# clysto/tinyimgcodec

Hardware: AMD Instinct MI355X
Metric: Mpixels/s encode (DCT+quant kernel) (higher is better)
Workload: dtype f32+f64

## Files before the change

tinyimgcodec_amd/csrc/tic_kernels.hip:

```cpp
#include <hip/hip_runtime.h>
#include <hip/hip_ext.h>
#include <stdint.h>
#include <stdlib.h>
#include <string.h>
#include <type_traits>

#include "tic_hooks.h"
#include "tic_kernels.h"
#include "tic_math.h"

namespace tic {

#define TIC_DPP_QP_XOR1 0xB1
#define TIC_DPP_QP_XOR2 0x4E
#define TIC_DPP_ROW_SHL4 0x104
#define TIC_DPP_ROW_SHR4 0x114

__device__ __forceinline__ uint32_t perm_b32(uint32_t hi_src, uint32_t lo_src, uint32_t sel) {
    return __builtin_amdgcn_perm(hi_src, lo_src, sel);
}

__device__ __forceinline__ void transpose8x8_bytes(uint32_t &lo, uint32_t &hi, int i) {
    uint32_t nhi = (uint32_t)__builtin_amdgcn_update_dpp((int)hi, (int)lo, TIC_DPP_ROW_SHL4, 0xf, 0x5, false);
    uint32_t nlo = (uint32_t)__builtin_amdgcn_update_dpp((int)lo, (int)hi, TIC_DPP_ROW_SHR4, 0xf, 0xa, false);
    lo = nlo;
    hi = nhi;
    uint32_t selB = (i & 2) ? 0x03020706u : 0x05040100u;
    uint32_t plo = (uint32_t)__builtin_amdgcn_mov_dpp((int)lo, TIC_DPP_QP_XOR2, 0xf, 0xf, true);
    uint32_t phi = (uint32_t)__builtin_amdgcn_mov_dpp((int)hi, TIC_DPP_QP_XOR2, 0xf, 0xf, true);
    lo = perm_b32(plo, lo, selB);
    hi = perm_b32(phi, hi, selB);
    uint32_t selC = (i & 1) ? 0x03070105u : 0x06020400u;
    plo = (uint32_t)__builtin_amdgcn_mov_dpp((int)lo, TIC_DPP_QP_XOR1, 0xf, 0xf, true);
    phi = (uint32_t)__builtin_amdgcn_mov_dpp((int)hi, TIC_DPP_QP_XOR1, 0xf, 0xf, true);
    lo = perm_b32(plo, lo, selC);
    hi = perm_b32(phi, hi, selC);
}

__device__ __forceinline__ void transpose8x8_bytes_shfl(uint32_t &lo, uint32_t &hi, int i) {
    uint32_t row[2] = {lo, hi};
    uint32_t col_lo = 0, col_hi = 0;
    int base = (threadIdx.x & 63) & ~7;
    for (int r = 0; r < 8; r++) {
        uint32_t l = __shfl(row[0], base + r, 64), h = __shfl(row[1], base + r, 64);
        uint32_t w = (i < 4) ? l : h;
        uint32_t byte = (w >> (8 * (i & 3))) & 0xffu;
        if (r < 4)
            col_lo |= byte << (8 * r);
        else
            col_hi |= byte << (8 * (r - 4));
    }
    lo = col_lo;
    hi = col_hi;
}

__device__ __forceinline__ void wave_lds_fence() {
    __builtin_amdgcn_fence(__ATOMIC_RELEASE, "wavefront");
    __builtin_amdgcn_wave_barrier();
    __builtin_amdgcn_fence(__ATOMIC_ACQUIRE, "wavefront");
}

__device__ __forceinline__ int reflect_index(int i, int n) {
    if (i < n) return i;
    if (n >= 8) return 2 * (n - 1) - i;
    if (n == 1) return 0;
    int p = 2 * (n - 1), j = i;
    while (j >= p) j -= p;
    return j < n ? j : p - j;
}

constexpr int kWavesPerWG = 4;
constexpr int kLdsStrideDw = 68;
constexpr int kZzStrideB = 144;
constexpr int kLdsWaveBytes = 8 * kLdsStrideDw * 4;

struct Strip {
    int by, bx;
    bool valid;
    size_t oblk;
};

__device__ __forceinline__ void load_block_row(const uint8_t *__restrict__ img, int h, int w, long stride, bool aligned8,
                                               const Strip &s, int i, uint32_t &lo, uint32_t &hi) {
    lo = 0;
    hi = 0;
    if (!s.valid) return;
    int y = reflect_index(s.by * 8 + i, h);
    int x0 = s.bx * 8;
    const uint8_t *p = img + (long)y * stride + x0;
    if (aligned8 && x0 + 8 <= w) {
        uint2 v = *reinterpret_cast<const uint2 *>(p);
        lo = v.x;
        hi = v.y;
    } else {
        const uint8_t *rowp = img + (long)y * stride;
#pragma unroll
        for (int k = 0; k < 8; k++) {
            uint32_t b = rowp[reflect_index(x0 + k, w)];
            if (k < 4)
                lo |= b << (8 * k);
            else
                hi |= b << (8 * (k - 4));
        }
    }
}

__device__ __forceinline__ void transpose8x8_dwords(uint32_t *lds, int b, int i, uint32_t v[8]) {
    uint32_t *blk = lds + b * kLdsStrideDw;
#pragma unroll
    for (int u = 0; u < 8; u++) blk[u * 8 + i] = v[u];
    wave_lds_fence();
    const uint4 *rp = reinterpret_cast<const uint4 *>(blk + i * 8);
    uint4 a = rp[0], c = rp[1];
    v[0] = a.x; v[1] = a.y; v[2] = a.z; v[3] = a.w;
    v[4] = c.x; v[5] = c.y; v[6] = c.z; v[7] = c.w;
    wave_lds_fence();
}

__device__ __forceinline__ void exact_block(uint32_t colLo, uint32_t colHi, uint32_t *lds, int b, int i,
                                         const DctqConsts *__restrict__ C, int q[8]) {
    double c[8];
#pragma unroll
    for (int r = 0; r < 4; r++) {
        c[r] = (double)((int)((colLo >> (8 * r)) & 0xffu) - 128);
        c[r + 4] = (double)((int)((colHi >> (8 * r)) & 0xffu) - 128);
    }
    dct8_exact(c[0], c[1], c[2], c[3], c[4], c[5], c[6], c[7]);
    uint32_t w[8];
#pragma unroll
    for (int k = 0; k < 8; k++) w[k] = (uint32_t)__double2loint(c[k]);
    transpose8x8_dwords(lds, b, i, w);
    uint32_t wh[8];
#pragma unroll
    for (int k = 0; k < 8; k++) wh[k] = (uint32_t)__double2hiint(c[k]);
    transpose8x8_dwords(lds, b, i, wh);
#pragma unroll
    for (int k = 0; k < 8; k++) c[k] = __hiloint2double((int)wh[k], (int)w[k]);
    dct8_exact(c[0], c[1], c[2], c[3], c[4], c[5], c[6], c[7]);
    const double *div = C->div + i * 8;
#pragma unroll
    for (int v = 0; v < 8; v++) {
        q[v] = (int)rint(c[v] / div[v]);
        __builtin_amdgcn_sched_barrier(0);
    }
}

__device__ __forceinline__ void store_zigzag(uint32_t *lds, int b, int i, const uint16_t zz[8], const int q[8],
                                             int16_t *__restrict__ out, const Strip &s) {
    char *blk = reinterpret_cast<char *>(lds) + b * kZzStrideB;
#pragma unroll
    for (int v = 0; v < 8; v++) *reinterpret_cast<int16_t *>(blk + zz[v]) = (int16_t)q[v];
    wave_lds_fence();
    uint4 val = *reinterpret_cast<const uint4 *>(blk + i * 16);
    wave_lds_fence();
    if (s.valid) *reinterpret_cast<uint4 *>(out + s.oblk * 64 + i * 8) = val;
}

__device__ __forceinline__ Strip make_strip(int tile, int ntiles, int tiles_x, int bw, int b) {
    Strip s;
    int ty = tile / tiles_x;
    int tx = tile - ty * tiles_x;
    s.by = ty;
    s.bx = tx * 8 + b;
    s.valid = (tile < ntiles) && (s.bx < bw);
    s.oblk = (size_t)ty * bw + s.bx;
    return s;
}

__global__ __launch_bounds__(kWavesPerWG * 64) void dctq_exact_kernel(DctqArgs a) {
    __shared__ __attribute__((aligned(16))) uint32_t lds_all[kWavesPerWG][kLdsWaveBytes / 4];
    a.img += (long)blockIdx.y * a.frame_stride_in;
    a.out = reinterpret_cast<int16_t *>(reinterpret_cast<char *>(a.out) + (long)blockIdx.y * a.frame_stride_out);
    const int lane = threadIdx.x & 63, wave = threadIdx.x >> 6;
    const int b = lane >> 3, i = lane & 7;
    uint32_t *lds = lds_all[wave];
    int tile = blockIdx.x * kWavesPerWG + wave;
    int ntiles = a.ntiles;
    if (a.rem_mode) {
        const int bh = a.ntiles / a.tiles_x, rw = a.tiles_x - a.fast_tx;
        const int n_right = bh * rw, n_bottom = (bh - a.fast_ty) * a.fast_tx;
        ntiles = 0;
        if (tile < n_right) {
            tile = (tile / rw) * a.tiles_x + a.fast_tx + tile % rw;
            ntiles = a.ntiles;
        } else if (tile < n_right + n_bottom) {
            const int k = tile - n_right;
            tile = (a.fast_ty + k / a.fast_tx) * a.tiles_x + k % a.fast_tx;
            ntiles = a.ntiles;
        }
    }
    Strip s = make_strip(tile, ntiles, a.tiles_x, a.bw, b);
    uint32_t lo, hi;
    load_block_row(a.img, a.h, a.w, a.stride, a.aligned8, s, i, lo, hi);
    transpose8x8_bytes(lo, hi, i);
    int q[8];
    exact_block(lo, hi, lds, b, i, a.consts, q);
    const uint4 zzv = *reinterpret_cast<const uint4 *>(a.consts->zzofs + i * 8);
    uint16_t zz[8] = {(uint16_t)zzv.x, (uint16_t)(zzv.x >> 16), (uint16_t)zzv.y, (uint16_t)(zzv.y >> 16),
                      (uint16_t)zzv.z, (uint16_t)(zzv.z >> 16), (uint16_t)zzv.w, (uint16_t)(zzv.w >> 16)};
    store_zigzag(lds, b, i, zz, q, a.out, s);
}

constexpr int kTWaveBytes = kLdsWaveBytes;
constexpr int kTHalfDw = 272;
constexpr int kZzWaveBytes = 8 * kZzStrideB;
constexpr int kPxBlkBytes = 80;
constexpr int kMaxStripsPerWave = 16;
constexpr int kChunkStrips = 8;

__device__ __forceinline__ void quant_fma(float z, float mul, uint32_t &bits, float &d) {
    const float s = fmaf(z, mul, kMagic);
    bits = __float_as_uint(s);
    const float nr = kMagic - s;
    d = fmaf(z, mul, nr);
}

__device__ __forceinline__ void store16_wt_nt(void *p, const uint4 &v) {
    typedef uint32_t u32x4 __attribute__((ext_vector_type(4)));
    const u32x4 d = {v.x, v.y, v.z, v.w};
    asm volatile("global_store_dwordx4 %0, %1, off sc1 nt" : : "v"(p), "v"(d) : "memory");
}
__device__ __forceinline__ void store16_wt_nt(const void *sbase, uint32_t voff, const uint4 &v) {
    typedef uint32_t u32x4 __attribute__((ext_vector_type(4)));
    const u32x4 d = {v.x, v.y, v.z, v.w};
    asm volatile("global_store_dwordx4 %0, %1, %2 sc1 nt" : : "v"(voff), "v"(d), "s"(sbase) : "memory");
}

constexpr int kMaxStripsPerWave2 = 64;
constexpr int kBatch = 8;
constexpr int kBatchWaveBytes = kBatch * (128 + 64) + 64;

template <int CTRL>
__device__ __forceinline__ double dpp_f64(double x) {
    const int lo = __builtin_amdgcn_mov_dpp(__double2loint(x), CTRL, 0xf, 0xf, true);
    const int hi = __builtin_amdgcn_mov_dpp(__double2hiint(x), CTRL, 0xf, 0xf, true);
    return __hiloint2double(hi, lo);
}

__device__ __forceinline__ int rational_quad(const uint32_t *ldsT, int b, int i, const double *cst_rat) {
#pragma clang fp contract(off)
    const int w = i >> 2, k = i & 3;
    const uint32_t ca = (0x05010300u >> (8 * k)) & 0xffu, cb = (0x06020407u >> (8 * k)) & 0xffu;
    const uint32_t *row = ldsT + w * 128 + 4 * b;
    const float fa = __uint_as_float(row[(ca >> 2) * kTHalfDw + (ca & 3)]);
    const float fb = __uint_as_float(row[(cb >> 2) * kTHalfDw + (cb & 3)]);
    const double K = w ? (kTW3 * 0.5) : (kSq2h * 0.5);
    const double ya = (double)fa * K, yb = (double)fb * K;
    const double p = ya + yb;
    const double s2 = p + dpp_f64<TIC_DPP_QP_XOR1>(p);
    const double o = dpp_f64<TIC_DPP_QP_XOR2>(s2);
    const double E = (k & 1) ? s2 - o : s2 + o;
    const double X = E * ((k & 1) ? (kTW3 * 0.5) : (kSq2h * 0.5));
    const double div = cst_rat[2 * w + (k & 1)], rdiv = cst_rat[4 + 2 * w + (k & 1)];
    return (int)rint(div_rn(X, div, rdiv));
}

__device__ __forceinline__ int rational_slim(uint32_t rowLo, uint32_t rowHi, int i, const double *cst_rat) {
#pragma clang fp contract(off)
    uint32_t lo = perm_b32(rowHi, rowLo, 0x04030700u);
    uint32_t hi = perm_b32(rowHi, rowLo, 0x06050201u);
    transpose8x8_bytes(lo, hi, i);
    const uint32_t tot = __builtin_amdgcn_sad_u8(lo, 0u, __builtin_amdgcn_sad_u8(hi, 0u, 0u));
    const uint32_t sa = __builtin_amdgcn_sad_u8(lo & 0xff0000ffu, 0u, __builtin_amdgcn_sad_u8(hi & 0xff0000ffu, 0u, 0u));
    const int e0 = (int)tot - 1024, e4 = 2 * (int)sa - (int)tot;
    double y0 = (double)e0 * (kSq2h * 0.5);
    double y4 = (double)e4 * (kTW3 * 0.5);
    y0 = y0 + dpp_f64<TIC_DPP_QP_XOR1>(y0);
    y4 = y4 + dpp_f64<TIC_DPP_QP_XOR1>(y4);
    y0 = y0 + dpp_f64<TIC_DPP_QP_XOR2>(y0);
    y4 = y4 + dpp_f64<TIC_DPP_QP_XOR2>(y4);
    const double b0 = dpp_f64<TIC_DPP_ROW_SHL4>(y0), b4 = dpp_f64<TIC_DPP_ROW_SHL4>(y4);
    const double A = (i & 2) ? y4 : y0, B = (i & 2) ? b4 : b0;
    const double E = (i & 1) ? A - B : A + B;
    const double X = E * ((i & 1) ? (kTW3 * 0.5) : (kSq2h * 0.5));
    const double div = cst_rat[i & 3], rdiv = cst_rat[4 + (i & 3)];
    return (int)rint(div_rn(X, div, rdiv));
}
__device__ __forceinline__ unsigned long long wave_redo_block(const uint8_t *px , double *tbuf ,
                                                              const double *cosm, const double *rdiv, const uint16_t *zzofs, int16_t *img16,
                                                              int lane) {
    const int u = lane >> 3, c = lane & 7;
    typedef double d2 __attribute__((ext_vector_type(2)));
    const d2 *mu = reinterpret_cast<const d2 *>(cosm + u * 8), *mc = reinterpret_cast<const d2 *>(cosm + c * 8);
    const d2 m0 = mu[0], m1 = mu[1], m2 = mu[2], m3 = mu[3];
    double x[8];
#pragma unroll
    for (int r = 0; r < 8; r++) x[r] = (double)((int)px[r * 8 + c] - 128);
    double ta = m0.x * x[0], tb = m0.y * x[1];
    ta = fma(m1.x, x[2], ta); tb = fma(m1.y, x[3], tb);
    ta = fma(m2.x, x[4], ta); tb = fma(m2.y, x[5], tb);
    ta = fma(m3.x, x[6], ta); tb = fma(m3.y, x[7], tb);
    tbuf[u * 8 + c] = ta + tb;
    const d2 n0 = mc[0], n1 = mc[1], n2 = mc[2], n3 = mc[3];
    wave_lds_fence();
    const d2 *tu = reinterpret_cast<const d2 *>(tbuf + u * 8);
    const d2 y0 = tu[0], y1 = tu[1], y2 = tu[2], y3 = tu[3];
    double xa = n0.x * y0.x, xb = n0.y * y0.y;
    xa = fma(n1.x, y1.x, xa); xb = fma(n1.y, y1.y, xb);
    xa = fma(n2.x, y2.x, xa); xb = fma(n2.y, y2.y, xb);
    xa = fma(n3.x, y3.x, xa); xb = fma(n3.y, y3.y, xb);
    const double X = xa + xb;
    const double tq = X * rdiv[lane], rq = rint(tq);
    const bool rational = (lane & 0x1b) == 0;
    const bool decided = fabs(tq - rq) < 0.5 - 1e-9;
    if (decided && !rational) img16[zzofs[lane] >> 1] = (int16_t)(int)rq;
    const unsigned long long und = __ballot(!decided && !rational);
    wave_lds_fence();
    return und;
}

__device__ __forceinline__ uint32_t second_level_8(uint32_t colLo, uint32_t colHi, uint32_t *lds, int b, int i, const double *mul64, int q[8]) {
    double c[8];
#pragma unroll
    for (int r = 0; r < 4; r++) {
        c[r] = (double)(int)((colLo >> (8 * r)) & 0xffu);
        c[r + 4] = (double)(int)((colHi >> (8 * r)) & 0xffu);
    }
    dct8_aan(c[0], c[1], c[2], c[3], c[4], c[5], c[6], c[7]);
    c[0] -= 1024.0;
    uint32_t w[8], wh[8];
#pragma unroll
    for (int k = 0; k < 8; k++) w[k] = (uint32_t)__double2loint(c[k]);
    transpose8x8_dwords(lds, b, i, w);
#pragma unroll
    for (int k = 0; k < 8; k++) wh[k] = (uint32_t)__double2hiint(c[k]);
    transpose8x8_dwords(lds, b, i, wh);
#pragma unroll
    for (int k = 0; k < 8; k++) c[k] = __hiloint2double((int)wh[k], (int)w[k]);
    dct8_aan(c[0], c[1], c[2], c[3], c[4], c[5], c[6], c[7]);
    uint32_t und = 0;
#pragma unroll
    for (int v = 0; v < 8; v++) {
        const double t = c[v] * mul64[i * 8 + v], r = rint(t);
        q[v] = (int)r;
        if (!(fabs(t - r) < 0.5 - 1e-9)) und |= 1u << v;
    }
    return und;
}

template <bool kCols>
__global__ __launch_bounds__(kWavesPerWG * 64, 6) __attribute__((amdgpu_num_vgpr(72))) void dctq_strip_kernel(DctqArgs a) {
    __shared__ __attribute__((aligned(16))) uint32_t ldsT_all[kWavesPerWG][kTWaveBytes / 4];
    __shared__ __attribute__((aligned(16))) uint32_t ldsZ_all[kWavesPerWG][kZzWaveBytes / 4];
    __shared__ __attribute__((aligned(16))) unsigned char cst_blk[kStripBlkBytes];
    __shared__ __attribute__((aligned(16))) uint32_t bat_all[kWavesPerWG][kBatchWaveBytes / 4];
    const int lane = threadIdx.x & 63;
    const int wave = __builtin_amdgcn_readfirstlane(threadIdx.x >> 6);
    uint32_t *ldsT = ldsT_all[wave];
    char *ldsZ = reinterpret_cast<char *>(ldsZ_all[wave]);
    const uint16_t *cst_zz = reinterpret_cast<const uint16_t *>(cst_blk + kBlkZz);
    const double *cst_rat = reinterpret_cast<const double *>(cst_blk + kBlkRat);
    uint4 *bat_img = reinterpret_cast<uint4 *>(bat_all[wave]);
    uint2 *bat_pix = reinterpret_cast<uint2 *>(bat_all[wave] + kBatch * 32);
    uint32_t *bat_id = bat_all[wave] + kBatch * 48;
    const DctqConsts *__restrict__ C = a.consts;
    a.img += (long)blockIdx.z * a.frame_stride_in;
    a.out = reinterpret_cast<int16_t *>(reinterpret_cast<char *>(a.out) + (long)blockIdx.z * a.frame_stride_out);

    const int lr = lane >> 3, lb = lane & 7;
    const int b = lane >> 3, i = lane & 7;
    unsigned long long mask_exact = 0;
    uint32_t n_second = 0, n_quad = 0;
    int nE = 0;
    int t_first, n_my;
    const uint32_t st_off = (uint32_t)lane * 16u;
    {
        typedef float f32x4 __attribute__((ext_vector_type(4)));
        typedef uint32_t u32x4 __attribute__((ext_vector_type(4)));
        f32x4 m0, m1;
        f32x4 thr;
        u32x4 zzv;
        u32x4 c_fill;
        {
            constexpr int kPpw = kStripBlkPieces / kWavesPerWG;
            static_assert(kPpw * kWavesPerWG == kStripBlkPieces && kPpw <= 64, "constant block must split evenly over the waves");
            const uint32_t piece = lane < kPpw ? (uint32_t)(wave * kPpw + lane) : (uint32_t)kStripBlkPieces - 1u;
            const uint32_t fo = piece * 16u;
            asm volatile("global_load_dwordx4 v[76:79], %0, %1" : : "v"(fo), "s"(C->strip_blk) : "memory", "v76", "v77", "v78", "v79");
        }
        const uint32_t px_wr = (uint32_t)(uintptr_t)(__attribute__((address_space(3))) char *)(ldsZ + lb * kPxBlkBytes + lr * 8);
        const uint8_t *px_rd = reinterpret_cast<const uint8_t *>(ldsZ + b * kPxBlkBytes + i);
        constexpr int kHalf = kCols ? kTHalfDw : 256;
        const int p1a = kCols ? i : lr, p1b = kCols ? b : lb;
        uint32_t *twA = ldsT + (p1a >> 2) * kHalf + (p1a & 3) + 4 * p1b;
        uint32_t *twB = ldsT + (p1a >> 2) * kHalf + (p1a & 3) + 4 * (p1b ^ 4);
        const uint4 *tr = reinterpret_cast<const uint4 *>(
            __builtin_assume_aligned(ldsT + i * 32 + 4 * (b ^ (4 * ((i >> 1) & 1))), 16));
        const uint32_t ld_off = (uint32_t)(lr * (int)a.stride + lb * 8);

        uint32_t tf, t_lim;
        if (a.team_count > 0) {
            const uint32_t r = blockIdx.y;
            const uint32_t row0 = (uint32_t)((r < 8u ? a.split_lo >> (8u * r) : a.split_hi) & 0xffull);
            const uint32_t row1 = (uint32_t)((r < 7u ? a.split_lo >> (8u * r + 8u) : a.split_hi) & 0xffull);
            tf = (row0 * (uint32_t)a.team_count + blockIdx.x) * kWavesPerWG + (uint32_t)wave;
            t_lim = tf + (row1 - row0) * (uint32_t)a.tstep;
        } else if (a.round_wgs > 0) {
            const uint32_t rho = a.magic_tstep ? __umulhi(blockIdx.x, a.magic_tstep ) : blockIdx.x;
            const uint32_t wl = blockIdx.x - rho * (uint32_t)a.round_wgs;
            const uint32_t base = rho * (uint32_t)a.round_wgs * (uint32_t)a.wg_span;
            tf = base + wl * kWavesPerWG + (uint32_t)wave;
            t_lim = base + (uint32_t)a.round_wgs * (uint32_t)a.wg_span;
        } else {
            tf = blockIdx.x * (uint32_t)a.wg_stride + (uint32_t)wave;
            t_lim = blockIdx.x * (uint32_t)a.wg_stride + (uint32_t)a.wg_span;
        }
        tf = __builtin_amdgcn_readfirstlane(tf);
        const uint32_t nfast = (uint32_t)a.fast_ty * (uint32_t)a.fast_tx;
        const uint32_t t_end = t_lim < nfast ? t_lim : nfast;
        n_my = 0;
        if (tf < t_end) n_my = (a.round_wgs > 0 || a.magic_tstep == 0u) ? (int)((t_end - tf + (uint32_t)a.tstep - 1u) / (uint32_t)a.tstep)
                                                                        : (int)__umulhi(t_end - tf + (uint32_t)a.tstep - 1u, a.magic_tstep);
        if (n_my == 0) tf = 0;
        t_first = (int)tf;
        const uint32_t ty_first = a.magic_fast_tx ? __umulhi(tf, a.magic_fast_tx) : tf;
        int txp = (int)(tf - ty_first * (uint32_t)a.fast_tx);
        uint32_t in_off = ty_first * (uint32_t)(8 * a.stride) + (uint32_t)txp * 64u;
        uint32_t oblk = ty_first * (uint32_t)a.bw + (uint32_t)txp * 8u;
        uint32_t src_off = 0;
        int n_issued = 0;
        const uint8_t *img_s = a.img;
#define TIC_RSV_CLOBBER "memory", "v72", "v73", "v74", "v75", "v76", "v77", "v78", "v79"
#define TIC_LOAD(R, OB)                                                                                      \
    do {                                                                                                     \
        src_off = n_issued < n_my ? in_off : src_off;                                                        \
        OB = oblk;                                                                                           \
        asm volatile("global_load_dwordx2 v[" R "], %0, %1" : : "v"(ld_off), "s"(img_s + src_off) : TIC_RSV_CLOBBER); \
        n_issued++; txp += a.step_tx; in_off += a.in_step32; oblk += a.oblk_step;                            \
        if (__builtin_expect(txp >= a.fast_tx, 0)) { txp -= a.fast_tx; in_off += a.in_wrap32; oblk += a.oblk_wrap; } \
    } while (0)
#define TIC_TAKE_COLS(R, N) asm volatile("s_waitcnt vmcnt(" #N ")\n\tds_write_b64 %0, v[" R "]" : : "v"(px_wr) : TIC_RSV_CLOBBER)
#define TIC_TAKE_ROWS(D, R0, R1, N)                                                                          \
    asm volatile("s_waitcnt vmcnt(" #N ")\n\tv_cvt_f32_ubyte0 %0, v" #R0 "\n\tv_cvt_f32_ubyte1 %1, v" #R0 "\n\tv_cvt_f32_ubyte2 %2, v" #R0 \
                 "\n\tv_cvt_f32_ubyte3 %3, v" #R0 "\n\tv_cvt_f32_ubyte0 %4, v" #R1 "\n\tv_cvt_f32_ubyte1 %5, v" #R1                       \
                 "\n\tv_cvt_f32_ubyte2 %6, v" #R1 "\n\tv_cvt_f32_ubyte3 %7, v" #R1                                                       \
                 : "=v"(D[0]), "=v"(D[1]), "=v"(D[2]), "=v"(D[3]), "=v"(D[4]), "=v"(D[5]), "=v"(D[6]), "=v"(D[7]) : : TIC_RSV_CLOBBER)
        uint32_t ob0, ob1, ob2;
        uint32_t kstrip = 0;
        TIC_LOAD("72:73", ob0);
        TIC_LOAD("74:75", ob1);
        asm volatile("s_waitcnt vmcnt(2)\n\tv_mov_b32 %0, v76\n\tv_mov_b32 %1, v77\n\tv_mov_b32 %2, v78\n\tv_mov_b32 %3, v79"
                     : "=v"(c_fill.x), "=v"(c_fill.y), "=v"(c_fill.z), "=v"(c_fill.w) : : "memory", "v76", "v77", "v78", "v79");
        if (lane < kStripBlkPieces / kWavesPerWG) *reinterpret_cast<u32x4 *>(cst_blk + (wave * (kStripBlkPieces / kWavesPerWG) + lane) * 16) = c_fill;
        asm volatile("s_waitcnt lgkmcnt(0)\n\ts_barrier" : : : "memory");
        m0 = *reinterpret_cast<const f32x4 *>(cst_blk + (kCols ? kBlkMul : kBlkMulT) + i * 32);
        m1 = *reinterpret_cast<const f32x4 *>(cst_blk + (kCols ? kBlkMul : kBlkMulT) + i * 32 + 16);
        thr = *reinterpret_cast<const f32x4 *>(cst_blk + (kCols ? kBlkThr : kBlkThrT) + i * 16);
        zzv = *reinterpret_cast<const u32x4 *>(cst_blk + (kCols ? kBlkZz : kBlkZzT) + i * 16);
        auto zz_ptr = [&](uint32_t ofs) {
            const uint32_t c = ofs >> 4;
            return reinterpret_cast<int16_t *>(ldsZ + c * 128 + (ofs & 15) + 16 * (b ^ (kCols ? (((c >> 1) & 1) | (c & 4)) : (4 * ((c >> 1) & 1)))));
        };
        int16_t *zp0 = zz_ptr(zzv.x & 0xffff), *zp1 = zz_ptr(zzv.x >> 16), *zp2 = zz_ptr(zzv.y & 0xffff), *zp3 = zz_ptr(zzv.y >> 16);
        int16_t *zp4 = zz_ptr(zzv.z & 0xffff), *zp5 = zz_ptr(zzv.z >> 16), *zp6 = zz_ptr(zzv.w & 0xffff), *zp7 = zz_ptr(zzv.w >> 16);
        const uint4 *zr = reinterpret_cast<const uint4 *>(
            __builtin_assume_aligned(ldsZ + 16 * (i * 8 + (b ^ (kCols ? (((i >> 1) & 1) | (i & 4)) : (4 * ((i >> 1) & 1))))), 16));
        wave_lds_fence();

        int left = n_my;
        auto raw_words = [&](auto tag, uint32_t &lo, uint32_t &hi) {
            constexpr int R = decltype(tag)::value;
            static_assert(R == 72 || R == 74 || R == 76, "landing register pair");
            if constexpr (R == 72) asm volatile("v_mov_b32 %0, v72\n\tv_mov_b32 %1, v73" : "=v"(lo), "=v"(hi) : : "memory");
            else if constexpr (R == 74) asm volatile("v_mov_b32 %0, v74\n\tv_mov_b32 %1, v75" : "=v"(lo), "=v"(hi) : : "memory");
            else asm volatile("v_mov_b32 %0, v76\n\tv_mov_b32 %1, v77" : "=v"(lo), "=v"(hi) : : "memory");
        };
        auto process = [&](auto tag, const float (&pxr)[8], const uint32_t ob) {
            float d0, d1, d2, d3, d4, d5, d6, d7;
            if constexpr (kCols) {
                d0 = (float)px_rd[0]; d1 = (float)px_rd[8]; d2 = (float)px_rd[16]; d3 = (float)px_rd[24];
                d4 = (float)px_rd[32]; d5 = (float)px_rd[40]; d6 = (float)px_rd[48]; d7 = (float)px_rd[56];
            } else {
                d0 = pxr[0]; d1 = pxr[1]; d2 = pxr[2]; d3 = pxr[3]; d4 = pxr[4]; d5 = pxr[5]; d6 = pxr[6]; d7 = pxr[7];
            }
            dct8_aan(d0, d1, d2, d3, d4, d5, d6, d7);
            d0 -= 1024.0f;
            twA[0 * 32] = __float_as_uint(d0); twA[1 * 32] = __float_as_uint(d1); twB[2 * 32] = __float_as_uint(d2);
            twB[3 * 32] = __float_as_uint(d3); twA[4 * 32] = __float_as_uint(d4); twA[5 * 32] = __float_as_uint(d5);
            twB[6 * 32] = __float_as_uint(d6); twB[7 * 32] = __float_as_uint(d7);
            wave_lds_fence();
            const uint4 ra = tr[0], rb = tr[kHalf / 4];
            wave_lds_fence();
            float e0 = __uint_as_float(ra.x), e1 = __uint_as_float(ra.y), e2 = __uint_as_float(ra.z), e3 = __uint_as_float(ra.w);
            float e4 = __uint_as_float(rb.x), e5 = __uint_as_float(rb.y), e6 = __uint_as_float(rb.z), e7 = __uint_as_float(rb.w);
            dct8_aan(e0, e1, e2, e3, e4, e5, e6, e7);
            uint32_t q0, q1, q2, q3, q4, q5, q6, q7;
            float r0, r1, r2, r3, r4, r5, r6, r7;
            quant_fma(e0, m0.x, q0, r0); quant_fma(e1, m0.y, q1, r1); quant_fma(e2, m0.z, q2, r2); quant_fma(e3, m0.w, q3, r3);
            quant_fma(e4, m1.x, q4, r4); quant_fma(e5, m1.y, q5, r5); quant_fma(e6, m1.z, q6, r6); quant_fma(e7, m1.w, q7, r7);
            const float mA1 = fmaxf(fmaxf(fabsf(r1), fabsf(r2)), fabsf(r3));
            const float mA2 = fmaxf(fmaxf(fabsf(r5), fabsf(r6)), fabsf(r7));
            const float mB = fmaxf(fabsf(r0), fabsf(r4));
            const unsigned long long cA = __ballot(mA1 > thr.x) | __ballot(mA2 > thr.y);
            const unsigned long long cB = __ballot(mB > thr.z);
            *zp0 = (int16_t)q0; *zp1 = (int16_t)q1; *zp2 = (int16_t)q2; *zp3 = (int16_t)q3;
            *zp4 = (int16_t)q4; *zp5 = (int16_t)q5; *zp6 = (int16_t)q6; *zp7 = (int16_t)q7;
            const unsigned long long kRat = 0x1111111111111111ull;
            if (__builtin_expect((cB & kRat) != 0ull, 0)) {
                n_quad++;
                if constexpr (kCols) {
                    const int rq = rational_quad(ldsT, b, i, cst_rat);
                    if ((i & 2) == 0) *zz_ptr(28u * (uint32_t)(i & 1) + 20u * (uint32_t)(i >> 2) + 30u * (uint32_t)((i & 1) & (i >> 2))) = (int16_t)rq;
                } else {
                    uint32_t lo0, hi0;
                    raw_words(tag, lo0, hi0);
                    uint2 *pb = reinterpret_cast<uint2 *>(ldsT);
                    pb[lb * 8 + lr] = make_uint2(lo0, hi0);
                    wave_lds_fence();
                    const uint2 rowv = pb[lane];
                    wave_lds_fence();
                    const int rq = rational_slim(rowv.x, rowv.y, i, cst_rat);
                    if (i < 4) *zz_ptr(i == 0 ? 0u : (i == 1 ? 28u : (i == 2 ? 20u : 78u))) = (int16_t)rq;
                }
            }
            wave_lds_fence();
            const uint4 val = *zr;
            wave_lds_fence();
            const char *dst = reinterpret_cast<const char *>(a.out) + ((unsigned long long)ob << 7);
            const unsigned long long mG = cA | (cB & ~kRat);
            if (__builtin_expect(mG != 0ull, 0)) {
                const uint32_t gm = (uint32_t)__ballot(((mG >> (8u * (uint32_t)i)) & 0xffull) != 0ull) & 0xffu;
                const int nnew = __builtin_popcount(gm);
                if (nE + nnew <= kBatch && gm != 0xffu) {
                    uint32_t lo0, hi0;
                    raw_words(tag, lo0, hi0);
                    const uint32_t below = (1u << b) - 1u, lbelow = (1u << lb) - 1u;
                    const bool mine = (gm >> b) & 1u;
                    const int e = nE + __builtin_popcount(gm & below);
                    if (mine) bat_img[e * 8 + i] = val;
                    if (mine && i == 0) bat_id[e] = ob + (uint32_t)b;
                    if ((gm >> lb) & 1u) bat_pix[(nE + __builtin_popcount(gm & lbelow)) * 8 + lr] = make_uint2(lo0, hi0);
                    if (!mine) store16_wt_nt(dst, st_off, val);
                    nE += nnew;
                    n_second += (uint32_t)nnew;
                } else {
                    mask_exact |= 1ull << kstrip;
                    store16_wt_nt(dst, st_off, val);
                }
            } else
                store16_wt_nt(dst, st_off, val);
            left--;
            kstrip++;
        };
        float pxf[8] = {0.f, 0.f, 0.f, 0.f, 0.f, 0.f, 0.f, 0.f};
#define TIC_STEP(RLOAD, OBL, RTAKE, R0, R1, OBP, N)                                                          \
        TIC_LOAD(RLOAD, OBL);                                                                                \
        if constexpr (kCols) { TIC_TAKE_COLS(RTAKE, N); } else { TIC_TAKE_ROWS(pxf, R0, R1, N); }            \
        process(std::integral_constant<int, R0>(), pxf, OBP)
        do {
            if (left == 0) break;
            TIC_STEP("76:77", ob2, "72:73", 72, 73, ob0, 2);
            if (left == 0) break;
            TIC_STEP("72:73", ob0, "74:75", 74, 75, ob1, 3);
            while (left != 0) {
                TIC_STEP("74:75", ob1, "76:77", 76, 77, ob2, 4);
                if (left == 0) break;
                TIC_STEP("76:77", ob2, "72:73", 72, 73, ob0, 4);
                if (left == 0) break;
                TIC_STEP("72:73", ob0, "74:75", 74, 75, ob1, 4);
            }
        } while (0);
#undef TIC_STEP
        asm volatile("; end of the strip walk" : : : TIC_RSV_CLOBBER);
#undef TIC_LOAD
#undef TIC_TAKE_COLS
#undef TIC_TAKE_ROWS
#undef TIC_RSV_CLOBBER
    }
    if (nE != 0) {
        const double *cst_cos = reinterpret_cast<const double *>(cst_blk + kBlkCos);
        const double *cst_rdiv = reinterpret_cast<const double *>(cst_blk + kBlkRdiv);
        uint32_t m_exact = 0;
        if (nE < 3) {
            for (int ee = 0; ee < nE; ee++) {
                const unsigned long long und = wave_redo_block(reinterpret_cast<const uint8_t *>(bat_pix + ee * 8), reinterpret_cast<double *>(ldsT), cst_cos,
                                                               cst_rdiv, cst_zz, reinterpret_cast<int16_t *>(bat_img + ee * 8), lane);
                if (und != 0ull) m_exact |= 1u << ee;
            }
        } else {
            const bool have2 = b < nE;
            const int e2 = have2 ? b : 0;
            const uint2 rowv = bat_pix[e2 * 8 + i];
            uint32_t lo = rowv.x, hi = rowv.y;
            transpose8x8_bytes(lo, hi, i);
            int qs[8];
            uint32_t und = second_level_8(lo, hi, ldsT, b, i, reinterpret_cast<const double *>(cst_blk + kBlkMul64), qs);
            if ((i & 3) == 0) und &= ~0x11u;
            const uint4 zo = *reinterpret_cast<const uint4 *>(cst_zz + i * 8);
            const uint32_t zw[4] = {zo.x, zo.y, zo.z, zo.w};
            int16_t *img2 = reinterpret_cast<int16_t *>(bat_img + e2 * 8);
            if (have2) {
#pragma unroll
                for (int v = 0; v < 8; v++)
                    if (!((und >> v) & 1u) && !((i & 3) == 0 && (v & 3) == 0)) img2[((zw[v >> 1] >> (16 * (v & 1))) & 0xffffu) >> 1] = (int16_t)qs[v];
            }
            const unsigned long long um = __ballot(have2 && und != 0u);
            for (int ee = 0; ee < nE; ee++)
                if ((um >> (8 * ee)) & 0xffull) m_exact |= 1u << ee;
        }
        const bool have = b < nE;
        const int e = have ? b : 0;
        const uint32_t blk = bat_id[e];
        if (m_exact != 0u) {
            const uint2 rowv = bat_pix[e * 8 + i];
            int16_t *img16 = reinterpret_cast<int16_t *>(bat_img + e * 8);
            uint32_t lo = rowv.x, hi = rowv.y;
            transpose8x8_bytes(lo, hi, i);
            const uint4 zo = *reinterpret_cast<const uint4 *>(cst_zz + i * 8);
            const uint32_t zw[4] = {zo.x, zo.y, zo.z, zo.w};
            int qx[8];
            exact_block(lo, hi, ldsT, b, i, C, qx);
            if (have && ((m_exact >> e) & 1u)) {
#pragma unroll
                for (int v = 0; v < 8; v++) img16[((zw[v >> 1] >> (16 * (v & 1))) & 0xffffu) >> 1] = (int16_t)qx[v];
            }
        }
        wave_lds_fence();
        const uint4 val = bat_img[e * 8 + i];
        if (have) store16_wt_nt(reinterpret_cast<char *>(a.out) + ((unsigned long long)blk << 7) + (uint32_t)i * 16u, val);
    }
    if (a.fallback_count != nullptr && lane == 0) {
        if (n_second != 0) atomicAdd(a.fallback_count, (unsigned long long)n_second);
        if (n_quad != 0) atomicAdd(a.fallback_count + 1, (unsigned long long)n_quad);
        if (mask_exact != 0ull) atomicAdd(a.fallback_count + 2, (unsigned long long)__builtin_popcountll(mask_exact));
        if (nE != 0) atomicMax(a.fallback_count + 3, (unsigned long long)nE);
    }
    if (mask_exact == 0ull) return;
    asm volatile("s_waitcnt vmcnt(0)" : : : "memory");
    const uint4 zzn = *reinterpret_cast<const uint4 *>(cst_zz + i * 8);
    const uint16_t zz[8] = {(uint16_t)zzn.x, (uint16_t)(zzn.x >> 16), (uint16_t)zzn.y, (uint16_t)(zzn.y >> 16),
                            (uint16_t)zzn.z, (uint16_t)(zzn.z >> 16), (uint16_t)zzn.w, (uint16_t)(zzn.w >> 16)};
    for (unsigned long long todo = mask_exact; todo != 0ull; todo &= todo - 1ull) {
        const int k = __builtin_ctzll(todo);
        const long t = (long)t_first + (long)k * a.tstep;
        const int ty = (int)(t / a.fast_tx), tx = (int)(t - (long)ty * a.fast_tx);
        Strip s;
        s.by = ty;
        s.bx = tx * 8 + b;
        s.valid = true;
        s.oblk = (size_t)ty * a.bw + s.bx;
        uint32_t lo, hi;
        load_block_row(a.img, a.h, a.w, a.stride, true, s, i, lo, hi);
        transpose8x8_bytes(lo, hi, i);
        int q[8];
        const uint32_t und = second_level_8(lo, hi, ldsT, b, i, reinterpret_cast<const double *>(cst_blk + kBlkMul64), q);
        if (__ballot(und != 0u) != 0ull) exact_block(lo, hi, ldsT, b, i, C, q);
        store_zigzag(reinterpret_cast<uint32_t *>(ldsZ), b, i, zz, q, a.out, s);
    }
}

__global__ __launch_bounds__(kWavesPerWG * 64) void dctq_exact_wide_kernel(WideArgs a) {
    __shared__ __attribute__((aligned(16))) uint32_t lds_all[kWavesPerWG][kLdsWaveBytes / 4];
    const int lane = threadIdx.x & 63, wave = threadIdx.x >> 6;
    const int b = lane >> 3, i = lane & 7;
    uint32_t *lds = lds_all[wave];
    const int tile = blockIdx.x * kWavesPerWG + wave;
    Strip s = make_strip(tile, a.ntiles, a.tiles_x, a.bw, b);
    double c[8];
#pragma unroll
    for (int r = 0; r < 8; r++) c[r] = 0.0;
    if (s.valid) {
        const int x = reflect_index(s.bx * 8 + i, a.w);
#pragma unroll
        for (int r = 0; r < 8; r++) {
            const int y = reflect_index(s.by * 8 + r, a.h);
            c[r] = (double)a.img[(long)y * a.stride + x] - 128.0;
        }
    }
    dct8_exact(c[0], c[1], c[2], c[3], c[4], c[5], c[6], c[7]);
    uint32_t w[8], wh[8];
#pragma unroll
    for (int k = 0; k < 8; k++) w[k] = (uint32_t)__double2loint(c[k]);
    transpose8x8_dwords(lds, b, i, w);
#pragma unroll
    for (int k = 0; k < 8; k++) wh[k] = (uint32_t)__double2hiint(c[k]);
    transpose8x8_dwords(lds, b, i, wh);
#pragma unroll
    for (int k = 0; k < 8; k++) c[k] = __hiloint2double((int)wh[k], (int)w[k]);
    dct8_exact(c[0], c[1], c[2], c[3], c[4], c[5], c[6], c[7]);
    if (!s.valid) return;
    const double *div = a.consts->div + i * 8;
    const uint16_t *zz = a.consts->zzofs + i * 8;
    int32_t *ob = a.out + s.oblk * 64;
#pragma unroll
    for (int v = 0; v < 8; v++) {
        ob[zz[v] >> 1] = (int32_t)rint(c[v] / div[v]);
        __builtin_amdgcn_sched_barrier(0);
    }
}

__constant__ int kAnnScalesInt[64] = {
    16384, 22725, 21407, 19266, 16384, 12873, 8867,  4520,  22725, 31521, 29692, 26722, 22725, 17855, 12299, 6270,
    21407, 29692, 27969, 25172, 21407, 16819, 11585, 5906,  19266, 26722, 25172, 22654, 19266, 15137, 10426, 5315,
    16384, 22725, 21407, 19266, 16384, 12873, 8867,  4520,  12873, 17855, 16819, 15137, 12873, 10114, 6967,  3552,
    8867,  12299, 11585, 10426, 8867,  6967,  4799,  2446,  4520,  6270,  5906,  5315,  4520,  3552,  2446,  1247};

template <bool kWideDc>
__device__ __forceinline__ void idct_body(const IdctArgs &a) {
    __shared__ __attribute__((aligned(16))) uint32_t lds_all[kWavesPerWG][kLdsWaveBytes / 4];
    const int lane = threadIdx.x & 63, wave = threadIdx.x >> 6;
    const int b = lane >> 3, i = lane & 7;
    uint32_t *lds = lds_all[wave];
    const int tile = blockIdx.x * kWavesPerWG + wave;
    const DctqConsts *__restrict__ C = a.consts;
    Strip s = make_strip(tile, a.ntiles, a.tiles_x, a.bw, b);
    if (a.first_block >= 0) {
        const long blk = a.first_block + (long)tile * 8 + b;
        s.valid = blk < a.first_block + a.nblocks_sel;
        s.by = (int)(blk / a.bw);
        s.bx = (int)(blk - (long)s.by * a.bw);
        s.oblk = (size_t)blk;
    }

    uint4 val = make_uint4(0, 0, 0, 0);
    if (s.valid) val = *reinterpret_cast<const uint4 *>(a.coeffs + s.oblk * 64 + i * 8);
    char *blk = reinterpret_cast<char *>(lds) + b * kZzStrideB;
    {
        uint32_t wv[4] = {val.x, val.y, val.z, val.w};
#pragma unroll
        for (int k = 0; k < 8; k++) {
            int nat = C->zznat[i * 8 + k];
            int16_t cv = (int16_t)((wv[k >> 1] >> (16 * (k & 1))) & 0xffffu);
            *reinterpret_cast<int16_t *>(blk + nat * 2) = cv;
        }
    }
    wave_lds_fence();
    double c[8];
#pragma unroll
    for (int u = 0; u < 8; u++) {
        int16_t cv = *reinterpret_cast<const int16_t *>(blk + (u * 8 + i) * 2);
        if (a.scaled)
            c[u] = (((double)cv / ((double)kAnnScalesInt[u * 8 + i] / 2048.0)) * a.pow2) * C->div[u * 8 + i];
        else
            c[u] = (double)cv * C->div[u * 8 + i];
    }
    if (kWideDc && i == 0 && s.valid) {
        const double dcv = (double)a.dc32[s.oblk];
        c[0] = a.scaled ? ((dcv / ((double)kAnnScalesInt[0] / 2048.0)) * a.pow2) * C->div[0] : dcv * C->div[0];
    }
    wave_lds_fence();
    idct8_exact(c[0], c[1], c[2], c[3], c[4], c[5], c[6], c[7]);
    uint32_t w[8], wh[8];
#pragma unroll
    for (int k = 0; k < 8; k++) w[k] = (uint32_t)__double2loint(c[k]);
    transpose8x8_dwords(lds, b, i, w);
#pragma unroll
    for (int k = 0; k < 8; k++) wh[k] = (uint32_t)__double2hiint(c[k]);
    transpose8x8_dwords(lds, b, i, wh);
#pragma unroll
    for (int k = 0; k < 8; k++) c[k] = __hiloint2double((int)wh[k], (int)w[k]);
    idct8_exact(c[0], c[1], c[2], c[3], c[4], c[5], c[6], c[7]);
    uint32_t px[8];
#pragma unroll
    for (int k = 0; k < 8; k++) {
        double v = c[k] + 128.0;
        v = v < 0.0 ? 0.0 : v;
        v = v > 255.0 ? 255.0 : v;
        px[k] = (uint32_t)(int)v;
    }
    if (!s.valid) return;
    int y = s.by * 8 + i;
    if (y >= a.h) return;
    int x0 = s.bx * 8;
    uint8_t *p = a.out + (long)y * a.stride + x0;
    if (a.aligned8 && x0 + 8 <= a.w) {
        uint2 o;
        o.x = px[0] | (px[1] << 8) | (px[2] << 16) | (px[3] << 24);
        o.y = px[4] | (px[5] << 8) | (px[6] << 16) | (px[7] << 24);
        *reinterpret_cast<uint2 *>(p) = o;
    } else {
#pragma unroll
        for (int k = 0; k < 8; k++)
            if (x0 + k < a.w) p[k] = (uint8_t)px[k];
    }
}
__global__ __launch_bounds__(kWavesPerWG * 64) void idct_kernel(IdctArgs a) { idct_body<false>(a); }
__global__ __launch_bounds__(kWavesPerWG * 64) void idct_wide_dc_kernel(IdctArgs a) { idct_body<true>(a); }

__global__ void selftest_transpose_kernel(const uint2 *in, uint2 *out_dpp, uint2 *out_ref) {
    int lane = threadIdx.x & 63, i = lane & 7;
    uint2 v = in[blockIdx.x * blockDim.x + threadIdx.x];
    uint32_t lo = v.x, hi = v.y;
    transpose8x8_bytes(lo, hi, i);
    out_dpp[blockIdx.x * blockDim.x + threadIdx.x] = make_uint2(lo, hi);
    lo = v.x;
    hi = v.y;
    transpose8x8_bytes_shfl(lo, hi, i);
    out_ref[blockIdx.x * blockDim.x + threadIdx.x] = make_uint2(lo, hi);
}

static inline int grid_for(int ntiles) { return (ntiles + kWavesPerWG - 1) / kWavesPerWG; }

struct Tunables {
    int max_wgs, sched, chunk, order;
    int split[8];
};
static Tunables read_tunables() {
    auto geti = [](const char *k, int d) { const char *v = test_hook(k); return v ? atoi(v) : d; };
    Tunables t;
    t.max_wgs = geti("TIC_MAX_WGS", 0);
    t.sched = geti("TIC_SCHED", 1);
    t.chunk = geti("TIC_CHUNK", kChunkStrips);
    t.order = geti("TIC_ORDER", -1);
    const char *sp = test_hook("TIC_SPLIT") ? test_hook("TIC_SPLIT") : "15,13,10,7,5,3";
    for (int k = 0; k < 8; k++) t.split[k] = 0;
    for (int k = 0; k < 8 && sp && *sp; k++) {
        t.split[k] = atoi(sp);
        sp = strchr(sp, ',');
        if (sp) sp++;
    }
    return t;
}
static Tunables tunables() {
    static const bool live = test_hook("TIC_TUNE") != nullptr;
    static const Tunables once = read_tunables();
    return live ? read_tunables() : once;
}

int dctq_kernel_id(int abi_variant) {
    return abi_variant == 1 ? 1 : ((abi_variant == 0 || abi_variant == 2) ? 2 : -1);
}

hipError_t launch_dctq(DctqArgs a, int variant, hipStream_t stream, hipEvent_t ev_start, hipEvent_t ev_stop) {
    if (a.ntiles <= 0) return hipSuccess;
    if (variant != 1 && variant != 2) return hipErrorInvalidValue;
    dim3 block(kWavesPerWG * 64);
    a.nwaves = a.step_ty = a.step_tx = 0;
    a.fast_ty = a.fast_tx = 0;
    a.rem_mode = 0;
    a.dbg = nullptr;
    const int nf = a.nframes > 0 ? a.nframes : 1;
    if (variant == 1) {
        hipLaunchKernelGGL(dctq_exact_kernel, dim3(grid_for(a.ntiles), nf), block, 0, stream, a);
        return hipGetLastError();
    }
    {
        long limit = 1L << 32;
        if (const char *e = test_hook("TIC_BAND_BYTES")) limit = atol(e) > 0 ? atol(e) : limit;
        if (a.aligned8 && nf == 1 && a.w >= 64 && (long)a.h * a.stride >= limit) {
            const long band = (limit - 1) / a.stride / 8 * 8;
            if (band >= 8) {
                for (long y0 = 0; y0 < a.h; y0 += band) {
                    DctqArgs b = a;
                    b.h = (int)((long)a.h - y0 < band ? (long)a.h - y0 : band);
                    b.img = a.img + y0 * a.stride;
                    b.out = a.out + (y0 / 8) * (long)a.bw * 64;
                    b.ntiles = ((b.h + 7) / 8) * b.tiles_x;
                    const hipError_t e = launch_dctq(b, variant, stream);
                    if (e != hipSuccess) return e;
                }
                return hipSuccess;
            }
        }
    }
    const int bh = a.ntiles / a.tiles_x;
    a.fast_tx = (a.aligned8 && (long)a.h * a.stride < (1L << 32)) ? a.w / 64 : 0;
    a.fast_ty = a.h / 8;
    const int nfast = a.fast_tx * a.fast_ty;
    if (nfast > 0) {
        const int max_strips = kMaxStripsPerWave2;
        int wgs = grid_for(nfast);
        static int cus = 256;
        static const int resident = [] {
            int dev = 0, per_cu = 0;
            hipDeviceProp_t prop;
            if (hipGetDevice(&dev) == hipSuccess && hipGetDeviceProperties(&prop, dev) == hipSuccess) cus = prop.multiProcessorCount;
            if (hipOccupancyMaxActiveBlocksPerMultiprocessor(&per_cu, dctq_strip_kernel<true>, kWavesPerWG * 64, 0) != hipSuccess || per_cu < 1)
                per_cu = 4;
            if (per_cu > 6) per_cu = 6;
            return cus * per_cu;
        }();
        const Tunables tune = tunables();
        const int cap_env = tune.max_wgs > 0 ? tune.max_wgs : resident;
        int cap = cap_env / nf;
        if (cap < 64) cap = 64;
        if (wgs > cap) wgs = cap;
        const int min_wgs = (nfast + kWavesPerWG * max_strips - 1) / (kWavesPerWG * max_strips);
        if (wgs < min_wgs) wgs = min_wgs;
        a.nwaves = wgs * kWavesPerWG;
        a.wg_stride = kWavesPerWG;
        a.tstep = a.nwaves;
        a.wg_span = nfast;
        a.round_wgs = 0;
        a.team_count = 0;
        const int S = tune.chunk < 1 ? 1 : (tune.chunk > max_strips ? max_strips : tune.chunk);
        const int min_wgs16 = (nfast + kWavesPerWG * kMaxStripsPerWave - 1) / (kWavesPerWG * kMaxStripsPerWave);
        const bool multi_round = (long)min_wgs16 * nf > (long)cap_env;
        if (tune.sched == 1 && multi_round) {
            a.wg_stride = a.wg_span = kWavesPerWG * S;
            a.tstep = kWavesPerWG;
            wgs = (nfast + a.wg_stride - 1) / a.wg_stride;
            a.nwaves = wgs * kWavesPerWG;
        } else if (tune.sched == 2 && multi_round && nf == 1) {
            a.round_wgs = cap_env;
            a.wg_span = kWavesPerWG * S;
            a.tstep = a.round_wgs * kWavesPerWG;
            wgs = (nfast + a.wg_span - 1) / a.wg_span;
            wgs = (wgs + a.round_wgs - 1) / a.round_wgs * a.round_wgs;
            a.nwaves = wgs * kWavesPerWG;
        }
        if (!multi_round && nf == 1 && tune.split[0] > 0 && wgs == cap_env && wgs % cus == 0 && wgs / cus <= 8) {
            const int R = wgs / cus;
            a.team_count = cus;
            a.tstep = cus * kWavesPerWG;
            const int rows_total = (nfast + a.tstep - 1) / a.tstep;
            double wsum = 0;
            for (int r = 0; r < R; r++) wsum += tune.split[r] > 0 ? tune.split[r] : 1;
            double acc = 0;
            a.split[0] = 0;
            for (int r = 0; r < R; r++) {
                acc += tune.split[r] > 0 ? tune.split[r] : 1;
                a.split[r + 1] = (int)(rows_total * acc / wsum + 0.5);
                if (a.split[r + 1] - a.split[r] > max_strips) a.team_count = 0;
            }
            a.split[R] = rows_total;
            if (rows_total > 255) a.team_count = 0;
            if (a.team_count == 0) a.tstep = a.nwaves;
        }
        a.step_ty = a.tstep / a.fast_tx;
        a.step_tx = a.tstep % a.fast_tx;
        a.in_step32 = (uint32_t)((long)a.step_ty * 8 * a.stride + (long)a.step_tx * 64);
        a.in_wrap32 = (uint32_t)(8 * a.stride - (long)a.fast_tx * 64);
        a.oblk_step = (uint32_t)((long)a.step_ty * a.bw + (long)a.step_tx * 8);
        a.oblk_wrap = (uint32_t)((long)a.bw - (long)a.fast_tx * 8);
        dim3 grid(wgs, 1, nf);
        const unsigned long long dmax = (unsigned long long)(a.round_wgs > 0 ? a.round_wgs : a.tstep);
        if ((unsigned long long)nfast * (unsigned long long)a.fast_tx >= (1ull << 32) ||
            ((unsigned long long)nfast + dmax) * dmax >= (1ull << 32)) {
            a.fast_tx = a.fast_ty = 0;
        } else {
            auto magic = [](long d) { return d <= 1 ? 0u : (uint32_t)((1ull << 32) / (unsigned long long)d + 1ull); };
            a.magic_fast_tx = magic(a.fast_tx);
            a.magic_tstep = magic(a.round_wgs > 0 ? a.round_wgs : a.tstep);
            a.split_lo = a.split_hi = 0;
            if (a.team_count > 0) {
                const int R = wgs / a.team_count;
                for (int k = 0; k <= R; k++) {
                    if (k < 8) a.split_lo |= (unsigned long long)(a.split[k] & 0xff) << (8 * k);
                    else a.split_hi = (unsigned long long)(a.split[k] & 0xff);
                }
                grid = dim3(a.team_count, R, nf);
            }
            const bool cols = tune.order < 0 ? !multi_round : tune.order == 1;
            if (ev_start && ev_stop) {
                if (cols)
                    hipExtLaunchKernelGGL(dctq_strip_kernel<true>, grid, block, 0, stream, ev_start, ev_stop, 0, a);
                else
                    hipExtLaunchKernelGGL(dctq_strip_kernel<false>, grid, block, 0, stream, ev_start, ev_stop, 0, a);
            } else if (cols)
                hipLaunchKernelGGL(dctq_strip_kernel<true>, grid, block, 0, stream, a);
            else
                hipLaunchKernelGGL(dctq_strip_kernel<false>, grid, block, 0, stream, a);
        }
    } else {
        a.fast_tx = a.fast_ty = 0;
    }
    const int nrem = bh * (a.tiles_x - a.fast_tx) + (bh - a.fast_ty) * a.fast_tx;
    if (nrem > 0) {
        a.rem_mode = 1;
        hipLaunchKernelGGL(dctq_exact_kernel, dim3(grid_for(nrem), nf), block, 0, stream, a);
    }
    return hipGetLastError();
}

hipError_t launch_dctq_wide(const WideArgs &a, hipStream_t stream) {
    if (a.ntiles <= 0) return hipSuccess;
    hipLaunchKernelGGL(dctq_exact_wide_kernel, dim3(grid_for(a.ntiles)), dim3(kWavesPerWG * 64), 0, stream, a);
    return hipGetLastError();
}

hipError_t launch_idct(const IdctArgs &a, hipStream_t stream) {
    if (a.ntiles <= 0) return hipSuccess;
    dim3 grid(grid_for(a.ntiles)), block(kWavesPerWG * 64);
    if (a.dc32) hipLaunchKernelGGL(idct_wide_dc_kernel, grid, block, 0, stream, a);
    else hipLaunchKernelGGL(idct_kernel, grid, block, 0, stream, a);
    return hipGetLastError();
}

hipError_t launch_selftest_transpose(const void *in, void *out_dpp, void *out_ref, int nthreads, hipStream_t stream) {
    hipLaunchKernelGGL(selftest_transpose_kernel, dim3(nthreads / 256), dim3(256), 0, stream, (const uint2 *)in,
                       (uint2 *)out_dpp, (uint2 *)out_ref);
    return hipGetLastError();
}

}
```

Measured before the change: 1.830 million.

## Replace split dword transposes with row-major double LDS transpose in fallback path

Rewrites the second-level fallback DCT so each lane starts from its row of pixels instead of a byte-transposed column. The intermediate doubles are transposed through LDS as whole doubles in two halves, and the half-pass is skipped when at most four blocks need it. The small-batch wave_redo_block path is removed in favour of always using the per-lane path. Output goes through a transposed zigzag table (kBlkZzT) and column-strided multipliers, which removes the byte transpose and the two 32-bit transposes, at the cost of extra LDS fences.

```diff
diff --git a/tinyimgcodec_amd/csrc/tic_kernels.hip b/tinyimgcodec_amd/csrc/tic_kernels.hip
--- a/tinyimgcodec_amd/csrc/tic_kernels.hip
+++ b/tinyimgcodec_amd/csrc/tic_kernels.hip
@@ -276,64 +276,43 @@
     const double div = cst_rat[i & 3], rdiv = cst_rat[4 + (i & 3)];
     return (int)rint(div_rn(X, div, rdiv));
 }
-__device__ __forceinline__ unsigned long long wave_redo_block(const uint8_t *px , double *tbuf ,
-                                                              const double *cosm, const double *rdiv, const uint16_t *zzofs, int16_t *img16,
-                                                              int lane) {
-    const int u = lane >> 3, c = lane & 7;
-    typedef double d2 __attribute__((ext_vector_type(2)));
-    const d2 *mu = reinterpret_cast<const d2 *>(cosm + u * 8), *mc = reinterpret_cast<const d2 *>(cosm + c * 8);
-    const d2 m0 = mu[0], m1 = mu[1], m2 = mu[2], m3 = mu[3];
-    double x[8];
-#pragma unroll
-    for (int r = 0; r < 8; r++) x[r] = (double)((int)px[r * 8 + c] - 128);
-    double ta = m0.x * x[0], tb = m0.y * x[1];
-    ta = fma(m1.x, x[2], ta); tb = fma(m1.y, x[3], tb);
-    ta = fma(m2.x, x[4], ta); tb = fma(m2.y, x[5], tb);
-    ta = fma(m3.x, x[6], ta); tb = fma(m3.y, x[7], tb);
-    tbuf[u * 8 + c] = ta + tb;
-    const d2 n0 = mc[0], n1 = mc[1], n2 = mc[2], n3 = mc[3];
-    wave_lds_fence();
-    const d2 *tu = reinterpret_cast<const d2 *>(tbuf + u * 8);
-    const d2 y0 = tu[0], y1 = tu[1], y2 = tu[2], y3 = tu[3];
-    double xa = n0.x * y0.x, xb = n0.y * y0.y;
-    xa = fma(n1.x, y1.x, xa); xb = fma(n1.y, y1.y, xb);
-    xa = fma(n2.x, y2.x, xa); xb = fma(n2.y, y2.y, xb);
-    xa = fma(n3.x, y3.x, xa); xb = fma(n3.y, y3.y, xb);
-    const double X = xa + xb;
-    const double tq = X * rdiv[lane], rq = rint(tq);
-    const bool rational = (lane & 0x1b) == 0;
-    const bool decided = fabs(tq - rq) < 0.5 - 1e-9;
-    if (decided && !rational) img16[zzofs[lane] >> 1] = (int16_t)(int)rq;
-    const unsigned long long und = __ballot(!decided && !rational);
-    wave_lds_fence();
-    return und;
-}
-
-__device__ __forceinline__ uint32_t second_level_8(uint32_t colLo, uint32_t colHi, uint32_t *lds, int b, int i, const double *mul64, int q[8]) {
+__device__ __forceinline__ uint32_t second_level_rows(uint32_t rowLo, uint32_t rowHi, uint32_t *lds, int b, int i, bool narrow,
+                                                      const double *mulcol , int q[8]) {
     double c[8];
 #pragma unroll
     for (int r = 0; r < 4; r++) {
-        c[r] = (double)(int)((colLo >> (8 * r)) & 0xffu);
-        c[r + 4] = (double)(int)((colHi >> (8 * r)) & 0xffu);
+        c[r] = (double)(int)((rowLo >> (8 * r)) & 0xffu);
+        c[r + 4] = (double)(int)((rowHi >> (8 * r)) & 0xffu);
     }
     dct8_aan(c[0], c[1], c[2], c[3], c[4], c[5], c[6], c[7]);
     c[0] -= 1024.0;
-    uint32_t w[8], wh[8];
-#pragma unroll
-    for (int k = 0; k < 8; k++) w[k] = (uint32_t)__double2loint(c[k]);
-    transpose8x8_dwords(lds, b, i, w);
-#pragma unroll
-    for (int k = 0; k < 8; k++) wh[k] = (uint32_t)__double2hiint(c[k]);
-    transpose8x8_dwords(lds, b, i, wh);
-#pragma unroll
-    for (int k = 0; k < 8; k++) c[k] = __hiloint2double((int)wh[k], (int)w[k]);
+    typedef double d2 __attribute__((ext_vector_type(2)));
+    static_assert(4 * kLdsStrideDw * 8 <= kLdsWaveBytes, "four blocks of doubles must fit the wave's transpose buffer");
+    double *blk = reinterpret_cast<double *>(lds) + (b & 3) * kLdsStrideDw;
+#pragma unroll
+    for (int h = 0; h < 2; h++) {
+        if (h == 1 && narrow) break;
+        const bool mine = (b >> 2) == h;
+        if (mine) {
+#pragma unroll
+            for (int v = 0; v < 8; v++) blk[v * 8 + i] = c[v];
+        }
+        wave_lds_fence();
+        if (mine) {
+            const d2 *rp = reinterpret_cast<const d2 *>(blk + i * 8);
+            const d2 y0 = rp[0], y1 = rp[1], y2 = rp[2], y3 = rp[3];
+            c[0] = y0.x; c[1] = y0.y; c[2] = y1.x; c[3] = y1.y;
+            c[4] = y2.x; c[5] = y2.y; c[6] = y3.x; c[7] = y3.y;
+        }
+        wave_lds_fence();
+    }
     dct8_aan(c[0], c[1], c[2], c[3], c[4], c[5], c[6], c[7]);
     uint32_t und = 0;
 #pragma unroll
-    for (int v = 0; v < 8; v++) {
-        const double t = c[v] * mul64[i * 8 + v], r = rint(t);
-        q[v] = (int)r;
-        if (!(fabs(t - r) < 0.5 - 1e-9)) und |= 1u << v;
+    for (int u = 0; u < 8; u++) {
+        const double t = c[u] * mulcol[u * 8], r = rint(t);
+        q[u] = (int)r;
+        if (!(fabs(t - r) < 0.5 - 1e-9)) und |= 1u << u;
     }
     return und;
 }
@@ -568,49 +547,32 @@
 #undef TIC_RSV_CLOBBER
     }
     if (nE != 0) {
-        const double *cst_cos = reinterpret_cast<const double *>(cst_blk + kBlkCos);
-        const double *cst_rdiv = reinterpret_cast<const double *>(cst_blk + kBlkRdiv);
-        uint32_t m_exact = 0;
-        if (nE < 3) {
-            for (int ee = 0; ee < nE; ee++) {
-                const unsigned long long und = wave_redo_block(reinterpret_cast<const uint8_t *>(bat_pix + ee * 8), reinterpret_cast<double *>(ldsT), cst_cos,
-                                                               cst_rdiv, cst_zz, reinterpret_cast<int16_t *>(bat_img + ee * 8), lane);
-                if (und != 0ull) m_exact |= 1u << ee;
-            }
-        } else {
-            const bool have2 = b < nE;
-            const int e2 = have2 ? b : 0;
-            const uint2 rowv = bat_pix[e2 * 8 + i];
-            uint32_t lo = rowv.x, hi = rowv.y;
-            transpose8x8_bytes(lo, hi, i);
-            int qs[8];
-            uint32_t und = second_level_8(lo, hi, ldsT, b, i, reinterpret_cast<const double *>(cst_blk + kBlkMul64), qs);
-            if ((i & 3) == 0) und &= ~0x11u;
-            const uint4 zo = *reinterpret_cast<const uint4 *>(cst_zz + i * 8);
-            const uint32_t zw[4] = {zo.x, zo.y, zo.z, zo.w};
-            int16_t *img2 = reinterpret_cast<int16_t *>(bat_img + e2 * 8);
-            if (have2) {
-#pragma unroll
-                for (int v = 0; v < 8; v++)
-                    if (!((und >> v) & 1u) && !((i & 3) == 0 && (v & 3) == 0)) img2[((zw[v >> 1] >> (16 * (v & 1))) & 0xffffu) >> 1] = (int16_t)qs[v];
-            }
-            const unsigned long long um = __ballot(have2 && und != 0u);
-            for (int ee = 0; ee < nE; ee++)
-                if ((um >> (8 * ee)) & 0xffull) m_exact |= 1u << ee;
-        }
         const bool have = b < nE;
         const int e = have ? b : 0;
+        const uint2 rowv = bat_pix[e * 8 + i];
         const uint32_t blk = bat_id[e];
-        if (m_exact != 0u) {
-            const uint2 rowv = bat_pix[e * 8 + i];
-            int16_t *img16 = reinterpret_cast<int16_t *>(bat_img + e * 8);
+        const uint4 zt = *reinterpret_cast<const uint4 *>(cst_blk + kBlkZzT + i * 16);
+        const double *mulc = reinterpret_cast<const double *>(cst_blk + kBlkMul64) + i;
+        int16_t *img16 = reinterpret_cast<int16_t *>(bat_img + e * 8);
+        int qs[8];
+        uint32_t und = second_level_rows(rowv.x, rowv.y, ldsT, b, i, nE <= 4, mulc, qs);
+        if ((i & 3) == 0) und &= ~0x11u;
+        if (have) {
+            const uint32_t zw[4] = {zt.x, zt.y, zt.z, zt.w};
+#pragma unroll
+            for (int u = 0; u < 8; u++)
+                if (!((und >> u) & 1u) && !((i & 3) == 0 && (u & 3) == 0)) img16[((zw[u >> 1] >> (16 * (u & 1))) & 0xffffu) >> 1] = (int16_t)qs[u];
+        }
+        const unsigned long long um = __ballot(have && und != 0u);
+        if (um != 0ull) {
+            const bool redo = ((um >> (8 * e)) & 0xffull) != 0ull;
             uint32_t lo = rowv.x, hi = rowv.y;
             transpose8x8_bytes(lo, hi, i);
             const uint4 zo = *reinterpret_cast<const uint4 *>(cst_zz + i * 8);
             const uint32_t zw[4] = {zo.x, zo.y, zo.z, zo.w};
             int qx[8];
             exact_block(lo, hi, ldsT, b, i, C, qx);
-            if (have && ((m_exact >> e) & 1u)) {
+            if (have && redo) {
 #pragma unroll
                 for (int v = 0; v < 8; v++) img16[((zw[v >> 1] >> (16 * (v & 1))) & 0xffffu) >> 1] = (int16_t)qx[v];
             }
@@ -627,9 +589,7 @@
     }
     if (mask_exact == 0ull) return;
     asm volatile("s_waitcnt vmcnt(0)" : : : "memory");
-    const uint4 zzn = *reinterpret_cast<const uint4 *>(cst_zz + i * 8);
-    const uint16_t zz[8] = {(uint16_t)zzn.x, (uint16_t)(zzn.x >> 16), (uint16_t)zzn.y, (uint16_t)(zzn.y >> 16),
-                            (uint16_t)zzn.z, (uint16_t)(zzn.z >> 16), (uint16_t)zzn.w, (uint16_t)(zzn.w >> 16)};
+    const double *mult = reinterpret_cast<const double *>(cst_blk + kBlkMul64) + i;
     for (unsigned long long todo = mask_exact; todo != 0ull; todo &= todo - 1ull) {
         const int k = __builtin_ctzll(todo);
         const long t = (long)t_first + (long)k * a.tstep;
@@ -641,11 +601,17 @@
         s.oblk = (size_t)ty * a.bw + s.bx;
         uint32_t lo, hi;
         load_block_row(a.img, a.h, a.w, a.stride, true, s, i, lo, hi);
-        transpose8x8_bytes(lo, hi, i);
         int q[8];
-        const uint32_t und = second_level_8(lo, hi, ldsT, b, i, reinterpret_cast<const double *>(cst_blk + kBlkMul64), q);
-        if (__ballot(und != 0u) != 0ull) exact_block(lo, hi, ldsT, b, i, C, q);
-        store_zigzag(reinterpret_cast<uint32_t *>(ldsZ), b, i, zz, q, a.out, s);
+        const uint32_t und = second_level_rows(lo, hi, ldsT, b, i, false, mult, q);
+        const bool ex = __ballot(und != 0u) != 0ull;
+        if (ex) {
+            transpose8x8_bytes(lo, hi, i);
+            exact_block(lo, hi, ldsT, b, i, C, q);
+        }
+        const uint4 zzn = *reinterpret_cast<const uint4 *>(cst_blk + (ex ? kBlkZz : kBlkZzT) + i * 16);
+        const uint16_t zsel[8] = {(uint16_t)zzn.x, (uint16_t)(zzn.x >> 16), (uint16_t)zzn.y, (uint16_t)(zzn.y >> 16),
+                                  (uint16_t)zzn.z, (uint16_t)(zzn.z >> 16), (uint16_t)zzn.w, (uint16_t)(zzn.w >> 16)};
+        store_zigzag(reinterpret_cast<uint32_t *>(ldsZ), b, i, zsel, q, a.out, s);
     }
 }
 
```

Result: slower. 1.711 million (-6.5%).
